# Roywangj/AdaptPoint

Measured on AMD Instinct MI355X. Metric: set-abstraction fwd+bwd point-clouds/sec (B=32,N=1024), higher is better.
Workload: dtype bf16

## Files before the change

### adaptpoint_amd/csrc/sa_fused.hip

```cpp
#include "apn_common.h"
#include "apn_mfma.h"
#include <type_traits>
#include "sa_chain.h"

namespace apn {

constexpr int SA_C = 32;
constexpr int SA_C1 = 32;
constexpr int SA_C2 = 64;
constexpr int SA_K = 32;
constexpr int SA_WAVES = 4;

template <int NS>
__device__ __forceinline__ void put_frag(uint4 *base, int f, int lane, const Frag<NS> &v) {
#pragma unroll
    for (int p = 0; p < NS; ++p) base[(f * NS + p) * 64 + lane] = __builtin_bit_cast(uint4, v.p[p]);
}

template <int NS>
__device__ __forceinline__ Frag<NS> get_frag(const uint4 *base, int f, int lane) {
    Frag<NS> v;
#pragma unroll
    for (int p = 0; p < NS; ++p) v.p[p] = __builtin_bit_cast(bf16x8, base[(f * NS + p) * 64 + lane]);
    return v;
// ... 305 lines not shown
            });
            stamp(a, wave, nst < 5 ? nst : 5);
            ++nst;
            hd_nxt = hd_nxt2;
            continue;
        }
        touch(hd_nxt);
        pre();
        if (more) fetch_tile<NS>(a, hd_nxt, h, nxt);
        const TileHead hd_nxt2 = load_head<CP>(a, tile2 < tiles ? tile2 : tile, r);
        body(tile, cur, nst == 4, [&] { touch(hd_nxt2); });
        stamp(a, wave, nst < 5 ? nst : 5);
        ++nst;
        if (more) cur = nxt;
        hd_nxt = hd_nxt2;
    }
    pre();
    stamp(a, wave, 6);
}

template <int NV>
__device__ __forceinline__ float fold_partials(float (&vals)[NV], int lane, int wave) {
    __shared__ float red[SA_WAVES][NV][32];
#pragma unroll
    for (int i = 0; i < NV; ++i) {
        const float other = __shfl_xor(vals[i], 32);
        if (lane < 32) red[wave][i][lane] = vals[i] + other;
    }
    __syncthreads();
    float s = 0.0f;
    const int e = threadIdx.x;
    if (e < NV * 32) {
#pragma unroll
        for (int w = 0; w < SA_WAVES; ++w) s += red[w][e >> 5][e & 31];
    }
    return s;
}

__device__ __forceinline__ void fold_rows32(const float *__restrict__ part, int rows, const double *__restrict__ sums,
                                            const BnArgs &bn, float *__restrict__ pack, float &scale, float &shift,
                                            double *scratch ) {
    double (*fred)[64] = reinterpret_cast<double (*)[64]>(scratch);
    double *ftot = scratch + 16 * 64;
    const int tid = threadIdx.x;
    double count = bn.count;
    double gpre = 1.0, bpre = 0.0;
    if (tid < 32) {
        if (bn.gamma) gpre = (double)bn.gamma[tid];
        if (bn.beta) bpre = (double)bn.beta[tid];
    }
    if (bn.training) {
        if (part) {
            const int quad = tid & 15, rg = tid >> 4;
            const float4 *__restrict__ p4 = reinterpret_cast<const float4 *>(part) + quad;
            double s0 = 0.0, s1 = 0.0, s2 = 0.0, s3 = 0.0;
            int rr = rg;
            for (; rr + 7 * 16 < rows; rr += 8 * 16) {
                float4 v[8];
#pragma unroll
                for (int u = 0; u < 8; ++u) v[u] = p4[(size_t)(rr + 16 * u) * 16];
#pragma unroll
                for (int u = 0; u < 8; ++u) {
                    s0 += (double)v[u].x; s1 += (double)v[u].y; s2 += (double)v[u].z; s3 += (double)v[u].w;
                }
            }
            for (; rr + 3 * 16 < rows; rr += 4 * 16) {
                float4 v[4];
#pragma unroll
                for (int u = 0; u < 4; ++u) v[u] = p4[(size_t)(rr + 16 * u) * 16];
#pragma unroll
                for (int u = 0; u < 4; ++u) {
                    s0 += (double)v[u].x; s1 += (double)v[u].y; s2 += (double)v[u].z; s3 += (double)v[u].w;
                }
            }
            for (; rr < rows; rr += 16) {
                const float4 v = p4[(size_t)rr * 16];
                s0 += (double)v.x; s1 += (double)v.y; s2 += (double)v.z; s3 += (double)v.w;
            }
            fred[rg][4 * quad] = s0; fred[rg][4 * quad + 1] = s1; fred[rg][4 * quad + 2] = s2; fred[rg][4 * quad + 3] = s3;
            __syncthreads();
            if (tid < 64) {
                double s = 0.0;
#pragma unroll
                for (int k = 0; k < 16; ++k) s += fred[k][tid];
                ftot[tid] = s;
            }
        } else if (tid < 64) {
            ftot[tid] = sums[tid];
        }
        if (!part) count = sums[64];
        __syncthreads();
    }
    if (tid < 32) {
        if (tid == 0 && blockIdx.x == 0 && bn.training && bn.nbt) *bn.nbt += 1;
        bn_channel(bn, 32, tid, bn.training ? ftot[tid] : 0.0, bn.training ? ftot[32 + tid] : 0.0, count,
                   blockIdx.x == 0, pack, scale, shift, gpre, bpre);
    }
}

template <int NS, bool CP>
__global__ __launch_bounds__(SA_WAVES * 64, 3) void sa_fwd_main_kernel(
    SaArgs a, const float *__restrict__ w2, BnArgs bn1, const float *__restrict__ part1, int rows1,
    const double *__restrict__ sums1, float *__restrict__ pack1, const float *__restrict__ gamma2,
    float *__restrict__ ysel, unsigned char *__restrict__ ksel, unsigned long long *__restrict__ acc2) {
    const int lane = threadIdx.x & 63, r = lane & 31, h = lane >> 5;
    const int wave = __builtin_amdgcn_readfirstlane(threadIdx.x >> 6);
    enum { F_W1 = 0, F_W2 = 3, F_COUNT = 7 };
    __shared__ uint4 cfrag[F_COUNT * NS * 64];
    __shared__ __attribute__((aligned(16))) float bn1v[2][2][16];
    constexpr int PT_WAVE = CP ? 2 * 32 * 33 : 17 * 64 * 2 / SA_WAVES;
    __shared__ __attribute__((aligned(16))) float ptile[SA_WAVES * PT_WAVE];
    __shared__ __attribute__((aligned(16))) unsigned sinfo[SA_WAVES][32];
    static_assert(SA_WAVES * PT_WAVE * 4 >= 17 * 64 * 8, "fold scratch");
    critical_stream_priority();
    stamp(a, wave, 0);
    const float sg[2] = {(!gamma2 || gamma2[r] >= 0.0f) ? 1.0f : -1.0f, (!gamma2 || gamma2[32 + r] >= 0.0f) ? 1.0f : -1.0f};
    float st[4] = {0.0f, 0.0f, 0.0f, 0.0f};

    auto prologue = [&]() {
        if (wave == 0) {
            Frag<NS> w1f[3];
            load_w1_frags<NS>(a.w1, r, h, w1f);
#pragma unroll
            for (int s = 0; s < 3; ++s) put_frag<NS>(cfrag, F_W1 + s, lane, w1f[s]);
        }
        if (wave == 1 || wave == 2) {
            const int t = wave - 1;
#pragma unroll
            for (int s = 0; s < 2; ++s) {
                float tmp[8];
#pragma unroll
                for (int j = 0; j < 8; ++j) tmp[j] = w2[(32 * t + r) * SA_C1 + acc_row(8 * s + j, h)];
                put_frag<NS>(cfrag, F_W2 + 2 * t + s, lane, make_frag<NS>(tmp));
            }
        }
        float sc, sh;
        fold_rows32(part1, rows1, sums1, bn1, pack1, sc, sh, reinterpret_cast<double *>(ptile));
        if (threadIdx.x < 32) {
            const int i = threadIdx.x;
            bn1v[0][(i >> 2) & 1][(i & 3) + 4 * (i >> 3)] = sc;
            bn1v[1][(i >> 2) & 1][(i & 3) + 4 * (i >> 3)] = sh;
        }
        __syncthreads();
    };

    for_each_tile<NS, CP>(a, wave, r, h, prologue, [] {}, [&](int tile, const TileRaw<NS> &raw, bool, auto before_stores) {
        int lane_o = lane;
        asm volatile("" : "+v"(lane_o));
        Frag<NS> x[3];
        build_frags<NS>(a, raw, h, x);
        const int q0 = __builtin_amdgcn_readfirstlane(raw.q0);
        const int nq = __builtin_amdgcn_readfirstlane((int)(raw.info >> 24));
        float multf[16];
        unsigned starts = 1u;
        float *pt = ptile + wave * PT_WAVE;
        if (CP) {
            if (lane < 32) sinfo[wave][lane] = raw.info;
#pragma unroll
            for (int gq = 0; gq < 4; ++gq) {
                const uint4 v = *reinterpret_cast<const uint4 *>(&sinfo[wave][8 * gq + 4 * (lane_o >> 5)]);
                multf[4 * gq] = (float)ri_mult(v.x); multf[4 * gq + 1] = (float)ri_mult(v.y);
                multf[4 * gq + 2] = (float)ri_mult(v.z); multf[4 * gq + 3] = (float)ri_mult(v.w);
            }
            const unsigned prev = (unsigned)__shfl_up((int)raw.info, 1);
            starts = (unsigned)__ballot(lane < 32 && (lane == 0 || ri_q(raw.info) != ri_q(prev)));
        }
        f32x16 y1 = {0};
#pragma unroll
        for (int s = 0; s < 3; ++s) y1 = mfma<NS>(get_frag<NS>(cfrag, F_W1 + s, lane_o), x[s], y1);
        {
            const float4 *scv = reinterpret_cast<const float4 *>(bn1v[0][lane_o >> 5]);
            const float4 *shv = reinterpret_cast<const float4 *>(bn1v[1][lane_o >> 5]);
#pragma unroll
            for (int i4 = 0; i4 < 4; ++i4) {
                const float4 sc = scv[i4], sh = shv[i4];
                y1[4 * i4] = __builtin_fmaxf(__builtin_fmaf(y1[4 * i4], sc.x, sh.x), 0.0f);
                y1[4 * i4 + 1] = __builtin_fmaxf(__builtin_fmaf(y1[4 * i4 + 1], sc.y, sh.y), 0.0f);
                y1[4 * i4 + 2] = __builtin_fmaxf(__builtin_fmaf(y1[4 * i4 + 2], sc.z, sh.z), 0.0f);
                y1[4 * i4 + 3] = __builtin_fmaxf(__builtin_fmaf(y1[4 * i4 + 3], sc.w, sh.w), 0.0f);
            }
        }
        const Frag<NS> a0 = pack8<NS>(y1, 0), a1 = pack8<NS>(y1, 8);
#pragma unroll
        for (int t = 0; t < 2; ++t) {
            f32x16 y2 = {0};
            y2 = mfma<NS>(a0, get_frag<NS>(cfrag, F_W2 + 2 * t, lane_o), y2);
            y2 = mfma<NS>(a1, get_frag<NS>(cfrag, F_W2 + 2 * t + 1, lane_o), y2);
            if (CP) {
                float s1 = 0.0f, s2 = 0.0f;
#pragma unroll
                for (int i = 0; i < 16; ++i) {
                    const float wy = multf[i] * y2[i];
                    s1 += wy;
                    s2 += wy * y2[i];
                    pt[(t * 32 + acc_row(i, h)) * 33 + r] = sg[t] * y2[i];
                }
                st[t] += s1;
                st[2 + t] += s2;
                continue;
            }
            float best = sg[t] * y2[0];
            int bpos = 0;
            float s1 = 0.0f, s2 = 0.0f;
#pragma unroll
            for (int i = 0; i < 16; ++i) {
                s1 += y2[i];
                s2 += y2[i] * y2[i];
                const float v = sg[t] * y2[i];
                if (i > 0 && v > best) { best = v; bpos = i; }
            }
            st[t] += s1;
            st[2 + t] += s2;
            int kpos = acc_row(bpos, h);
            const float obest = __shfl_xor(best, 32);
            const int okpos = __shfl_xor(kpos, 32);
            if (obest > best || (obest == best && okpos < kpos)) { best = obest; kpos = okpos; }
            if (h == 0) {
                ysel[(size_t)tile * SA_C2 + 32 * t + r] = sg[t] * best;
                ksel[(size_t)tile * SA_C2 + 32 * t + r] = (unsigned char)kpos;
            }
        }
        if (CP) {
            asm volatile("" ::: "memory");
            const float *mine = pt + h * (32 * 33) + r;
            const float sgn = h ? sg[1] : sg[0];
            float *ys = ysel + (size_t)q0 * SA_C2 + lane;
            unsigned char *ks = ksel + (size_t)q0 * SA_C2 + lane;
            before_stores();
            int seg = -1, ra = 0, kpos = 0;
            float best = 0.0f;
#pragma unroll
            for (int half16 = 0; half16 < 2; ++half16) {
                float v[16];
#pragma unroll
                for (int i = 0; i < 16; ++i) v[i] = mine[(16 * half16 + i) * 33];
#pragma unroll
                for (int i = 0; i < 16; ++i) {
                    const int rho = 16 * half16 + i;
                    if ((starts >> rho) & 1u) {
                        if (seg >= 0 && seg < nq) {
                            ys[(size_t)seg * SA_C2] = sgn * best;
                            ks[(size_t)seg * SA_C2] = (unsigned char)kpos;
                        }
                        ++seg;
                        best = -__builtin_inff();
                        kpos = 0;
                        ra = rho;
                    }
                    const bool up = v[i] > best;
                    best = up ? v[i] : best;
                    kpos = up ? rho - ra : kpos;
                }
            }
            if (seg >= 0 && seg < nq) {
                ys[(size_t)seg * SA_C2] = sgn * best;
                ks[(size_t)seg * SA_C2] = (unsigned char)kpos;
            }
            asm volatile("" ::: "memory");
        }
    });
    const float tot = fold_partials<4>(st, lane, wave);
    if (threadIdx.x < 128) acc_add(acc2, 128, blockIdx.x % ACC_COPIES, threadIdx.x, tot);
    stamp(a, wave, 7);
}

struct SaBwdArgs {
    const float *w2;
    const float *scale1, *shift1, *mean1, *inv1;
    const float *pack2;
    const unsigned long long *accS;
    const double *sumsS;
    double count;
    int train2;
    const float *goa;
    const unsigned char *ksel;
    const int *rowdst;
};

template <int NS, bool CP>
__global__ __launch_bounds__(SA_WAVES * 64, 2) void sa_bwd_kernel(SaArgs a, SaBwdArgs g,
                                                               unsigned long long *__restrict__ accT,
                                                               float *__restrict__ partW2,
                                                               float *__restrict__ GU,
                                                               float *__restrict__ HA,
                                                               float *__restrict__ HB) {
    static_assert(CP, "the backward pass runs over a tile map");
    const int lane = threadIdx.x & 63, r = lane & 31, h = lane >> 5;
    const int wave = __builtin_amdgcn_readfirstlane(threadIdx.x >> 6);
    enum { F_W1 = 0, F_QM = 3, F_W2T = 5, F_COUNT = 9 };
    __shared__ uint4 cfrag[F_COUNT * NS * 64];
    __shared__ __attribute__((aligned(16))) float bn1v[2][2][16];
    __shared__ __attribute__((aligned(16))) float sw2[SA_C2][SA_C1 + 4];
    __shared__ float sD[SA_C2], sE[SA_C2];
    __shared__ __attribute__((aligned(16))) float sqm[SA_C1 + 1][SA_C1 + 4];
    critical_stream_priority();
    stamp(a, wave, 0);
    __shared__ float chan[5][32];
    f32x16 dsp[2] = {{0}, {0}};
    f32x16 gram = {0};
    float suma = 0.0f;
    float st[2] = {0.0f, 0.0f};

    constexpr int SP_ROW = 72, SP_TILE = 32 * SP_ROW;
    constexpr int SP_WAVE = (CP && NS * SP_TILE * 2 < 2 * 32 * 33 * 4) ? 2 * 32 * 33 * 4 : NS * SP_TILE * 2;
    constexpr int SP_BYTES = SA_WAVES * SP_WAVE, WRED_BYTES = SA_WAVES * SA_C2 * SA_C1 * 4;
    __shared__ __attribute__((aligned(16))) unsigned char sp_raw[SP_BYTES > WRED_BYTES ? SP_BYTES : WRED_BYTES];
    __shared__ __attribute__((aligned(16))) unsigned sinfo[SA_WAVES][32];
    __shared__ __attribute__((aligned(16))) float qgoa[CP ? SA_WAVES : 1][4 * SA_C2];
    __shared__ __attribute__((aligned(16))) unsigned char qksel[CP ? SA_WAVES : 1][4 * SA_C2];
    __bf16 *sp_img = reinterpret_cast<__bf16 *>(sp_raw + wave * SP_WAVE);

    __shared__ __attribute__((aligned(16))) int sdst[SA_WAVES][2][64];
    int ahead_n = 0, body_n = 0;
    auto gu_store = [&](int place, float v) {
        *reinterpret_cast<float *>(reinterpret_cast<char *>(GU) + (((unsigned)place << 7) + ((unsigned)r << 2))) = v;
    };

    auto prologue = [&]() {
        const int tid = threadIdx.x;
        {
            Frag<NS> w1f[3];
            if (wave == 0) load_w1_frags<NS>(a.w1, r, h, w1f);
            float wv[8];
#pragma unroll
            for (int k = 0; k < 8; ++k) wv[k] = g.w2[tid + 256 * k];
            float c1[4] = {0.f, 0.f, 0.f, 0.f};
            if (tid >= 128 && tid < 160) {
                c1[0] = g.scale1[tid - 128]; c1[1] = g.shift1[tid - 128]; c1[2] = g.mean1[tid - 128]; c1[3] = g.inv1[tid - 128];
            }
            double sv = 0.0, count = g.count;
            float p_sc = 0.0f, p_mu = 0.0f, p_iv = 0.0f;
            if (tid < 128) sv = g.sumsS ? g.sumsS[tid] : acc_read(g.accS, 128, tid);
            if (g.sumsS) count = g.sumsS[128];
            if (tid < 64) { p_sc = g.pack2[tid]; p_mu = g.pack2[128 + tid]; p_iv = g.pack2[192 + tid]; }
            if (wave == 0) {
#pragma unroll
                for (int s = 0; s < 3; ++s) put_frag<NS>(cfrag, F_W1 + s, lane, w1f[s]);
            }
#pragma unroll
            for (int k = 0; k < 8; ++k) sw2[(tid + 256 * k) >> 5][tid & 31] = wv[k];
            if (tid >= 128 && tid < 160) {
#pragma unroll
                for (int k = 0; k < 4; ++k) chan[k][tid - 128] = c1[k];
            }
            double *sS2 = reinterpret_cast<double *>(&sqm[0][0]);
            if (tid >= 64 && tid < 128) sS2[tid - 64] = sv;
            __syncthreads();
            if (tid < 64) {
                const double sc = p_sc, mu = p_mu, iv = p_iv, s1 = sv, s2 = sS2[tid];
                double d = 0.0, e = 0.0;
                if (g.train2) {
                    const double rc = 1.0 / count;
                    d = -sc * iv * s2 * rc;
                    e = (-sc * s1 + sc * mu * iv * s2) * rc;
                }
                sD[tid] = (float)d;
                sE[tid] = (float)e;
            }
            if (tid >= 64 && tid < 96) {
                const int i = tid - 64;
                const float sci = g.scale1[i], shi = g.shift1[i];
                bn1v[0][(i >> 2) & 1][(i & 3) + 4 * (i >> 3)] = sci;
                bn1v[1][(i >> 2) & 1][(i & 3) + 4 * (i >> 3)] = shi;
            }
        }
        __syncthreads();
        {
            const int s = wave;
            float tmp[8], tmpd[8], tmpe[8];
#pragma unroll
            for (int j = 0; j < 8; ++j) {
                const int c = 16 * s + 8 * h + j;
                tmp[j] = sw2[c][r];
                tmpd[j] = tmp[j] * sD[c];
                tmpe[j] = r == 0 ? sE[c] : 0.0f;
            }
            const Frag<NS> wt = make_frag<NS>(tmp);
            put_frag<NS>(cfrag, F_W2T + s, lane, wt);
            const f32x16 zero16 = {0};
            const f32x16 qp = mfma<NS>(make_frag<NS>(tmpd), wt, zero16);
            const f32x16 ep = mfma<NS>(make_frag<NS>(tmpe), wt, zero16);
            float *scr = reinterpret_cast<float *>(sp_img);
#pragma unroll
            for (int e = 0; e < 16; ++e) scr[e * 64 + lane] = qp[e];
            if (h == 0) scr[16 * 64 + r] = ep[0];
        }
        __syncthreads();
        if (wave == 2) {
            f32x16 qacc = {0};
            float ev = 0.0f;
#pragma unroll
            for (int w = 0; w < SA_WAVES; ++w) {
                const float *pw = reinterpret_cast<const float *>(sp_raw + w * SP_WAVE);
#pragma unroll
                for (int e = 0; e < 16; ++e) qacc[e] += pw[e * 64 + lane];
                if (h == 0) ev += pw[16 * 64 + r];
            }
            put_frag<NS>(cfrag, F_QM, lane, pack8<NS>(qacc, 0));
            put_frag<NS>(cfrag, F_QM + 1, lane, pack8<NS>(qacc, 8));
            if (h == 0) chan[4][r] = ev;
        }
        __syncthreads();
        {
            uint4 *z = reinterpret_cast<uint4 *>(sp_img);
            for (int e = lane; e < SP_WAVE / 16; e += 64) z[e] = make_uint4(0u, 0u, 0u, 0u);
        }
    };

    auto scatter_pending = [] {};
    auto ahead = [&](const TileHead &hd) {
        if (!CP) return;
        typedef __attribute__((address_space(3))) void lds_void;
        typedef __attribute__((address_space(1))) const void glb_void;
        const int q0n = __builtin_amdgcn_readfirstlane(hd.q0);
        const int qbn = q0n < a.b * a.m - 4 ? q0n : a.b * a.m - 4;
        int l_o = lane;
        asm volatile("" : "+v"(l_o));
        const char *gb = reinterpret_cast<const char *>(g.goa) + (size_t)qbn * (SA_C2 * 4);
        const char *kb = reinterpret_cast<const char *>(g.ksel) + (size_t)qbn * SA_C2;
        __builtin_amdgcn_global_load_lds((glb_void *)(gb + (unsigned)(16 * l_o)), (lds_void *)&qgoa[wave][0], 16, 0, 0);
        __builtin_amdgcn_global_load_lds((glb_void *)(kb + (unsigned)(4 * l_o)), (lds_void *)&qksel[wave][0], 4, 0, 0);
        const char *db = reinterpret_cast<const char *>(g.rowdst) + (size_t)__builtin_amdgcn_readfirstlane(hd.tile) * (SA_K * 4);
        __builtin_amdgcn_global_load_lds((glb_void *)(db + (unsigned)(4 * (l_o & 31))), (lds_void *)&sdst[wave][ahead_n & 1][0], 4, 0, 0);
        ++ahead_n;
    };
    for_each_tile<NS, CP, CP>(a, wave, r, h, prologue, scatter_pending, [&](int tile, const TileRaw<NS> &raw, bool probe, auto before_stores) {
        auto st2 = [&](int k) { if (probe) stamp(a, wave, 8 + k); };
        st2(0);
        int lane_o = lane;
        asm volatile("" : "+v"(lane_o));
        Frag<NS> x[3];
        build_frags<NS>(a, raw, h, x);

        const int q0 = __builtin_amdgcn_readfirstlane(raw.q0);
        const int nq = CP ? __builtin_amdgcn_readfirstlane((int)(raw.info >> 24)) : 1;
        const bool live_row = !CP || ri_mult(raw.info) != 0;
        const float mrow = CP ? (float)ri_mult(raw.info) : 1.0f;
        float gv4[4];
        int kc4[4];
        const int qb = q0 < a.b * a.m - 4 ? q0 : a.b * a.m - 4;
#pragma unroll
        for (int u = 0; u < 4; ++u) {
            if (CP) {
                gv4[u] = 0.0f;
                kc4[u] = 0;
            } else {
                gv4[u] = 0.0f;
                kc4[u] = 0;
                if (u == 0) {
                    gv4[u] = g.goa[(size_t)(q0 + u) * SA_C2 + lane];
                    kc4[u] = g.ksel[(size_t)(q0 + u) * SA_C2 + lane];
                }
            }
        }
        unsigned mpk[4] = {0x01010101u, 0x01010101u, 0x01010101u, 0x01010101u};
        unsigned starts = 1u;
        if (CP) {
            if (lane < 32) sinfo[wave][lane] = raw.info;
#pragma unroll
            for (int gq = 0; gq < 4; ++gq) {
                const uint4 v = *reinterpret_cast<const uint4 *>(&sinfo[wave][8 * gq + 4 * (lane_o >> 5)]);
                mpk[gq] = ri_mult(v.x) | (ri_mult(v.y) << 8) | (ri_mult(v.z) << 16) | (ri_mult(v.w) << 24);
            }
            const unsigned prev = (unsigned)__shfl_up((int)raw.info, 1);
            starts = (unsigned)__ballot(lane < 32 && (lane == 0 || ri_q(raw.info) != ri_q(prev)));
        }
        auto multf = [&](int i) { return (float)((mpk[i >> 2] >> (8 * (i & 3))) & 0xffu); };
        f32x16 yT = {0}, y1 = {0};
#pragma unroll
        for (int s = 0; s < 3; ++s) {
            const Frag<NS> w = get_frag<NS>(cfrag, F_W1 + s, lane_o);
            yT = mfma<NS>(w, x[s], yT);
            y1 = mfma<NS>(x[s], w, y1);
        }
        {
            const float4 *scv = reinterpret_cast<const float4 *>(bn1v[0][lane_o >> 5]);
            const float4 *shv = reinterpret_cast<const float4 *>(bn1v[1][lane_o >> 5]);
#pragma unroll
            for (int i4 = 0; i4 < 4; ++i4) {
                const float4 sc = scv[i4], sh = shv[i4];
                yT[4 * i4] = __builtin_fmaxf(__builtin_fmaf(yT[4 * i4], sc.x, sh.x), 0.0f);
                yT[4 * i4 + 1] = __builtin_fmaxf(__builtin_fmaf(yT[4 * i4 + 1], sc.y, sh.y), 0.0f);
                yT[4 * i4 + 2] = __builtin_fmaxf(__builtin_fmaf(yT[4 * i4 + 2], sc.z, sh.z), 0.0f);
                yT[4 * i4 + 3] = __builtin_fmaxf(__builtin_fmaf(yT[4 * i4 + 3], sc.w, sh.w), 0.0f);
            }
        }
        st2(1);
        Frag<NS> a0, a1;
        if (CP) {
            f32x16 yw;
#pragma unroll
            for (int i = 0; i < 16; ++i) yw[i] = yT[i] * mrow;
            a0 = pack8<NS>(yw, 0);
            a1 = pack8<NS>(yw, 8);
        } else {
            a0 = pack8<NS>(yT, 0);
            a1 = pack8<NS>(yT, 8);
        }

        Frag<NS> sp[4];
        {
            unsigned todo = starts;
            if (CP) {
                asm volatile("s_waitcnt vmcnt(0)" ::: "memory");
                const int dq = q0 - qb;
#pragma unroll
                for (int u = 0; u < 4; ++u) {
                    const int e = (u + dq < 4 ? u + dq : 3) * SA_C2 + lane_o;
                    gv4[u] = qgoa[wave][e];
                    kc4[u] = qksel[wave][e];
                }
            }
#pragma unroll 1
            for (int jb = 0; jb < nq; jb += 4) {
                if (jb) {
#pragma unroll
                    for (int u = 0; u < 4; ++u)
                        if (jb + u < nq) {
                            gv4[u] = g.goa[(size_t)(q0 + jb + u) * SA_C2 + lane];
                            kc4[u] = g.ksel[(size_t)(q0 + jb + u) * SA_C2 + lane];
                        }
                }
#pragma unroll
                for (int u = 0; u < 4; ++u) {
                    if (jb + u < nq) {
                        const float gv = gv4[u];
                        int kc = kc4[u];
                        if (CP) {
                            kc += __builtin_ctz(todo);
                            todo &= todo - 1u;
                        }
                        const __bf16 ghi = (__bf16)gv;
                        const __bf16 glo = (__bf16)(gv - (float)ghi);
                        __bf16 *cell = sp_img + kc * SP_ROW + lane;
                        cell[0] = ghi;
                        if (NS == 2) cell[SP_TILE] = glo;
                        if (!CP) kc4[u] = kc;
                    }
                }
            }
        }
        asm volatile("" ::: "memory");
        {
            f32x16 an;
            const float sc1 = chan[0][lane_o & 31], sh1 = chan[1][lane_o & 31];
#pragma unroll
            for (int i = 0; i < 16; ++i) {
                an[i] = __builtin_fmaxf(__builtin_fmaf(y1[i], sc1, sh1), 0.0f);
                if (CP) suma = __builtin_fmaf(multf(i), an[i], suma);
                else suma += an[i];
            }
            const Frag<NS> b0 = pack8<NS>(an, 0), b1 = pack8<NS>(an, 8);
            if (CP) {
                f32x16 aw;
#pragma unroll
                for (int i = 0; i < 16; ++i) aw[i] = an[i] * multf(i);
                gram = mfma<NS>(pack8<NS>(aw, 0), b0, gram);
                gram = mfma<NS>(pack8<NS>(aw, 8), b1, gram);
            } else {
                gram = mfma<NS>(b0, b0, gram);
                gram = mfma<NS>(b1, b1, gram);
            }
            typedef short tr_s4 __attribute__((ext_vector_type(4)));
            typedef short tr_s8 __attribute__((ext_vector_type(8)));
            typedef __attribute__((address_space(3))) tr_s4 tr_lds;
            const int li = lane_o & 15, gq = li >> 2, gp = li & 3, grh = (lane_o >> 4) & 1;
            const __bf16 *tb = sp_img + (4 * (lane_o >> 5) + gq) * SP_ROW + 16 * grh + 4 * gp;
#pragma unroll
            for (int t = 0; t < 2; ++t) {
#pragma unroll
                for (int sk = 0; sk < 2; ++sk) {
                    Frag<NS> at;
#pragma unroll
                    for (int pp = 0; pp < NS; ++pp) {
                        const __bf16 *src = tb + pp * SP_TILE + (16 * sk) * SP_ROW + 32 * t;
                        const tr_s4 lo4 = __builtin_amdgcn_ds_read_tr16_b64_v4i16((tr_lds *)(src));
                        const tr_s4 hi4 = __builtin_amdgcn_ds_read_tr16_b64_v4i16((tr_lds *)(src + 8 * SP_ROW));
                        const tr_s8 v8 = {lo4.x, lo4.y, lo4.z, lo4.w, hi4.x, hi4.y, hi4.z, hi4.w};
                        at.p[pp] = __builtin_bit_cast(bf16x8, v8);
                    }
                    dsp[t] = mfma<NS>(at, sk ? b1 : b0, dsp[t]);
                }
            }
        }
        st2(2);
#pragma unroll
        for (int s = 0; s < 4; ++s) {
            const __bf16 *src = sp_img + r * SP_ROW + 16 * s + 8 * h;
            sp[s].p[0] = *reinterpret_cast<const bf16x8 *>(src);
            if (NS == 2) sp[s].p[NS - 1] = *reinterpret_cast<const bf16x8 *>(src + SP_TILE);
        }
        asm volatile("" ::: "memory");
        if (!CP) {
            __bf16 *cell = sp_img + kc4[0] * SP_ROW + lane;
            cell[0] = (__bf16)0.0f;
            if (NS == 2) cell[SP_TILE] = (__bf16)0.0f;
        }
        f32x16 ga;
        const float ev = chan[4][lane_o & 31];
#pragma unroll
        for (int i = 0; i < 16; ++i) ga[i] = CP ? ev * multf(i) : ev;
        ga = mfma<NS>(a0, get_frag<NS>(cfrag, F_QM, lane_o), ga);
        ga = mfma<NS>(a1, get_frag<NS>(cfrag, F_QM + 1, lane_o), ga);
#pragma unroll
        for (int s = 0; s < 4; ++s) ga = mfma<NS>(sp[s], get_frag<NS>(cfrag, F_W2T + s, lane_o), ga);

        st2(3);
        float *gt = reinterpret_cast<float *>(sp_img);
        asm volatile("" ::: "memory");
        float s1 = 0.0f, s2 = 0.0f, hb = 0.0f;
        const float sc1l = chan[0][lane_o & 31], sh1l = chan[1][lane_o & 31], iv1 = chan[3][lane_o & 31];
        const float nmi = -chan[2][lane_o & 31] * iv1;
#pragma unroll
        for (int i = 0; i < 16; ++i) {
            const float u = __builtin_fmaf(y1[i], sc1l, sh1l);
            const float yhat = __builtin_fmaf(y1[i], iv1, nmi);
            ga[i] = u > 0.0f ? ga[i] : 0.0f;
            s1 += ga[i];
            s2 += ga[i] * yhat;
            if (CP) {
                gt[acc_row(i, h) * 33 + r] = ga[i];
                gt[32 * 33 + acc_row(i, h) * 33 + r] = multf(i) * yhat;
            } else {
                hb += yhat;
            }
        }
        st[0] += s1;
        st[1] += s2;

        st2(4);
        before_stores();
        {
            int live;
            if (CP) {
                asm volatile("" ::: "memory");
                const float *mine = gt + h * (32 * 33) + r;
                float *dst = (h ? HB : HA) + (size_t)q0 * SA_C1 + r;
                int seg = -1;
                float sum = 0.0f;
#pragma unroll
                for (int half16 = 0; half16 < 2; ++half16) {
                    float v[16];
#pragma unroll
                    for (int i = 0; i < 16; ++i) v[i] = mine[(16 * half16 + i) * 33];
#pragma unroll
                    for (int i = 0; i < 16; ++i) {
                        if ((starts >> (16 * half16 + i)) & 1u) {
                            if (seg >= 0 && seg < nq) dst[(size_t)seg * SA_C1] = sum;
                            ++seg;
                            sum = 0.0f;
                        }
                        sum += v[i];
                    }
                }
                if (seg >= 0 && seg < nq) dst[(size_t)seg * SA_C1] = sum;
                asm volatile("" ::: "memory");
                {
                    uint4 *z = reinterpret_cast<uint4 *>(sp_img);
#pragma unroll
                    for (int e = 0; e < (NS * SP_TILE * 2 / 16 + 63) / 64; ++e)
                        if (e * 64 + lane < NS * SP_TILE * 2 / 16) z[e * 64 + lane] = make_uint4(0u, 0u, 0u, 0u);
                }
                asm volatile("" ::: "memory");
                live = __popcll(__ballot(lane < 32 && live_row));
            } else {
                const float ha = s1 + __shfl_xor(s1, 32);
                hb += __shfl_xor(hb, 32);
                if (h == 0) {
                    HA[(size_t)tile * SA_C1 + r] = ha;
                    HB[(size_t)tile * SA_C1 + r] = hb;
                }
                live = 0;
            }

            st2(5);
            st2(6);
            if (CP) {
                const int *dl = &sdst[wave][body_n & 1][0];
#pragma unroll
                for (int gq = 0; gq < 4; ++gq) {
                    if (8 * gq < live) {
                        const int4 dd = *reinterpret_cast<const int4 *>(&dl[8 * gq + 4 * (lane_o >> 5)]);
                        const int base = 8 * gq + 4 * h;
                        if (base + 0 < live) gu_store(dd.x, ga[4 * gq + 0]);
                        if (base + 1 < live) gu_store(dd.y, ga[4 * gq + 1]);
                        if (base + 2 < live) gu_store(dd.z, ga[4 * gq + 2]);
                        if (base + 3 < live) gu_store(dd.w, ga[4 * gq + 3]);
                    }
                }
            }
            ++body_n;
        }
    }, ahead);
    {
        const float tot = fold_partials<2>(st, lane, wave);
        if (threadIdx.x < 64) acc_add(accT, 64, blockIdx.x % ACC_COPIES, threadIdx.x, tot);
    }
    float (*wred)[SA_C2 * SA_C1] = reinterpret_cast<float (*)[SA_C2 * SA_C1]>(sp_raw);
    __syncthreads();
#pragma unroll
    for (int i = 0; i < 16; ++i) {
        wred[wave][acc_row(i, h) * SA_C1 + r] = dsp[0][i];
        wred[wave][(32 + acc_row(i, h)) * SA_C1 + r] = dsp[1][i];
    }
    __syncthreads();
    const int ec = threadIdx.x >> 2, emid = (threadIdx.x & 3) * 8;
    float sp8[8];
    {
        float4 lo4 = make_float4(0.f, 0.f, 0.f, 0.f), hi4 = lo4;
#pragma unroll
        for (int w = 0; w < SA_WAVES; ++w) {
            const float4 a4 = *reinterpret_cast<const float4 *>(&wred[w][ec * SA_C1 + emid]);
            const float4 b4 = *reinterpret_cast<const float4 *>(&wred[w][ec * SA_C1 + emid + 4]);
            lo4.x += a4.x; lo4.y += a4.y; lo4.z += a4.z; lo4.w += a4.w;
            hi4.x += b4.x; hi4.y += b4.y; hi4.z += b4.z; hi4.w += b4.w;
        }
        sp8[0] = lo4.x; sp8[1] = lo4.y; sp8[2] = lo4.z; sp8[3] = lo4.w;
        sp8[4] = hi4.x; sp8[5] = hi4.y; sp8[6] = hi4.z; sp8[7] = hi4.w;
    }
    __syncthreads();
    suma += __shfl_xor(suma, 32);
#pragma unroll
    for (int i = 0; i < 16; ++i) wred[wave][acc_row(i, h) * SA_C1 + r] = gram[i];
    if (h == 0) wred[wave][SA_C1 * SA_C1 + r] = suma;
    __syncthreads();
    for (int e = threadIdx.x; e < SA_C1 * SA_C1 + SA_C1; e += SA_WAVES * 64)
        sqm[e >> 5][e & 31] = (wred[0][e] + wred[1][e]) + (wred[2][e] + wred[3][e]);
    __syncthreads();
    {
        float acc[8];
#pragma unroll
        for (int j = 0; j < 8; ++j) acc[j] = 0.0f;
#pragma unroll 8
        for (int k = 0; k < SA_C1; ++k) {
            const float w = sw2[ec][k];
            const float4 g0 = *reinterpret_cast<const float4 *>(&sqm[k][emid]);
            const float4 g1 = *reinterpret_cast<const float4 *>(&sqm[k][emid + 4]);
            acc[0] = __builtin_fmaf(w, g0.x, acc[0]); acc[1] = __builtin_fmaf(w, g0.y, acc[1]);
            acc[2] = __builtin_fmaf(w, g0.z, acc[2]); acc[3] = __builtin_fmaf(w, g0.w, acc[3]);
            acc[4] = __builtin_fmaf(w, g1.x, acc[4]); acc[5] = __builtin_fmaf(w, g1.y, acc[5]);
            acc[6] = __builtin_fmaf(w, g1.z, acc[6]); acc[7] = __builtin_fmaf(w, g1.w, acc[7]);
        }
        const float d = sD[ec], e = sE[ec];
        const float4 s0 = *reinterpret_cast<const float4 *>(&sqm[32][emid]);
        const float4 s1 = *reinterpret_cast<const float4 *>(&sqm[32][emid + 4]);
        float4 *row = reinterpret_cast<float4 *>(partW2 + (size_t)blockIdx.x * (SA_C2 * SA_C1) + ec * SA_C1 + emid);
        row[0] = make_float4(sp8[0] + d * acc[0] + e * s0.x, sp8[1] + d * acc[1] + e * s0.y,
                             sp8[2] + d * acc[2] + e * s0.z, sp8[3] + d * acc[3] + e * s0.w);
        row[1] = make_float4(sp8[4] + d * acc[4] + e * s1.x, sp8[5] + d * acc[5] + e * s1.y,
                             sp8[6] + d * acc[6] + e * s1.z, sp8[7] + d * acc[7] + e * s1.w);
    }
    stamp(a, wave, 7);
}

static int sa_grid(int tiles, bool compact = false) {
    const int cap = compact ? 768 : 512;
    int g = (tiles + SA_WAVES - 1) / SA_WAVES;
    return g < cap ? (g < 1 ? 1 : g) : cap;
}

static int sa_grid_bwd(int tiles) {
    int g = sa_grid(tiles);
    return g < 448 ? g : 448;
}

}

extern "C" int apn_sa_grid_blocks(int b, int m) { return apn::sa_grid(b * m); }
extern "C" int apn_sa_grid_rows(int b, int m, int with_tile_map) { return apn::sa_grid(b * m, with_tile_map != 0); }
extern "C" int apn_sa_bwd_main_rows(int b, int m) { return apn::sa_grid_bwd(b * m); }
extern "C" int apn_sa_acc_words(int ncol) { return ncol > 0 ? apn::acc_words(ncol) : 0; }

extern "C" int apn_sa_prep_rows(int b, int n) {
    const long long tiles = (long long)b * ((n + apn::PS_PTS - 1) / apn::PS_PTS);
    return (int)(tiles < apn::PS_MAX_ROWS ? (tiles < 1 ? 1 : tiles) : apn::PS_MAX_ROWS);
}

extern "C" int apn_sa_prep_stats(int b, int n, const float *f, const void *geo, const void *dd, const float *w1,
                                 int precision, int stats, void *ft, float *part1, void *zero, long long zero_words,
                                 void *stream) {
    using namespace apn;
    if (b <= 0 || n <= 0 || b > 65535 || (precision != 1 && precision != 2) || !f || !ft || !w1) return APN_EINVAL;
    if (stats && (!geo || !dd || !part1 || ((uintptr_t)geo & 15) || ((uintptr_t)part1 & 15))) return APN_EINVAL;
    if (zero_words < 0 || (zero_words && !zero)) return APN_EINVAL;
    __bf16 *hi = (__bf16 *)ft;
    __bf16 *lo = precision == 2 ? hi + (size_t)b * n * SA_C : nullptr;
    const int tpc = (n + PS_PTS - 1) / PS_PTS;
    auto kern = precision == 2 ? sa_prep_stats_kernel<2> : sa_prep_stats_kernel<1>;
    const int lds = SA_C * (PS_PTS + 1) * (int)sizeof(float);
    static DynLdsOnce lds_set[2];
    if (hipError_t e = set_dyn_lds(lds_set[precision - 1], (const void *)kern, lds)) return (int)e;
    hipLaunchKernelGGL(kern, dim3(apn_sa_prep_rows(b, n)), dim3(PS_NT), lds, (hipStream_t)stream, n, tpc, b * tpc, f,
                       (const long long *)geo, (const double *)dd, b * (apn_sa_geo_dd_doubles(n) / 6), w1, stats, hi, lo, part1,
                       (unsigned long long *)zero, zero_words);
    APN_LAUNCH_CHECK();
    return APN_OK;
}

#ifdef APN_WG_STAMPS
extern "C" __attribute__((visibility("default"))) int apn_sa_debug_wg_stamps_fused(void *buf) {
    return (int)hipMemcpyToSymbol(HIP_SYMBOL(apn::d_wg_stamps_f), &buf, sizeof(buf));
}
#endif

static unsigned long long *g_stamps = nullptr;
extern "C" int apn_sa_debug_stamps(void *buf) { g_stamps = (unsigned long long *)buf; return APN_OK; }

static apn::SaArgs sa_args(int b, int n, int m, const float *xyz, const float *new_xyz, const void *ft,
                           int precision, const int *idx, const float *w1, float radius, const int *tmap) {
    const __bf16 *hi = (const __bf16 *)ft;
    return apn::SaArgs{b, n, m, xyz, new_xyz, hi,
                       precision == 2 ? hi + (size_t)b * n * apn::SA_C : nullptr, idx, w1, radius, tmap, g_stamps};
}

static int sa_check(int b, int n, int m, int precision) {
    if (precision != 1 && precision != 2) return APN_EINVAL;
    if (b <= 0 || n <= 0 || m <= 0) return APN_EINVAL;
    if ((long long)b * m > 0x7fffffffLL / 64) return APN_EINVAL;
    if ((long long)b * n > 0xffffffffLL / 256) return APN_EINVAL;
    if ((long long)b * m > 0xffffffffLL / (32 * 128)) return APN_EINVAL;
    return APN_OK;
}

extern "C" int apn_sa_fwd_main(int b, int n, int m, int precision, float radius, const float *xyz,
                               const float *new_xyz, const void *ft, const int *idx, const int *tmap, const float *w1,
                               const float *w2, const float *g1, const float *b1, float *rm1, float *rv1, void *nbt1,
                               float eps1, float mom1, int train1, double count, const float *part1, int rows1,
                               const double *sums1, float *pack1, const float *gamma2, float *ysel, void *ksel,
                               void *acc2, void *stream) {
    using namespace apn;
    if (int e = sa_check(b, n, m, precision)) return e;
    if (!xyz || !new_xyz || !ft || !idx || !w1 || !w2 || !pack1 || !ysel || !ksel || !acc2) return APN_EINVAL;
    if (train1 && !part1 && !sums1) return APN_EINVAL;
    if (!train1 && (!rm1 || !rv1)) return APN_EINVAL;
    if (part1 && (((uintptr_t)part1 & 15) || rows1 <= 0)) return APN_EINVAL;
    SaArgs a = sa_args(b, n, m, xyz, new_xyz, ft, precision, idx, w1, radius, tmap);
    BnArgs bn{g1, b1, rm1, rv1, (long long *)nbt1, eps1, mom1, train1, count};
    auto kern = precision == 2 ? (tmap ? sa_fwd_main_kernel<2, true> : sa_fwd_main_kernel<2, false>)
                               : (tmap ? sa_fwd_main_kernel<1, true> : sa_fwd_main_kernel<1, false>);
    hipLaunchKernelGGL(kern, dim3(sa_grid(b * m, tmap != nullptr)), dim3(SA_WAVES * 64), 0, (hipStream_t)stream, a, w2, bn,
                       sums1 ? nullptr : part1, rows1, sums1, pack1, gamma2, ysel, (unsigned char *)ksel,
                       (unsigned long long *)acc2);
    APN_LAUNCH_CHECK();
    return APN_OK;
}

extern "C" int apn_sa_bwd_main(int b, int n, int m, int precision, float radius, const float *xyz,
                               const float *new_xyz, const void *ft, const int *idx, const int *tmap, const float *w1,
                               const float *w2, const float *pack1, const float *pack2, const void *accS,
                               const double *sumsS, double count, int train2, const float *goa, const void *ksel,
                               void *accT, float *partW2, const int *rowdst, float *GU, float *HA, float *HB, void *stream) {
    using namespace apn;
    if (int e = sa_check(b, n, m, precision)) return e;
    if (!w2 || !pack1 || !pack2 || (!accS && !sumsS) || !goa || !ksel || !accT || !partW2 || !GU || !HA || !HB)
        return APN_EINVAL;
    if (!tmap || !rowdst) return APN_EINVAL;
    SaArgs a = sa_args(b, n, m, xyz, new_xyz, ft, precision, idx, w1, radius, tmap);
    SaBwdArgs g;
    g.w2 = w2;
    g.scale1 = pack1; g.shift1 = pack1 + 32; g.mean1 = pack1 + 64; g.inv1 = pack1 + 96;
    g.pack2 = pack2;
    g.accS = (const unsigned long long *)accS; g.sumsS = sumsS;
    g.count = count; g.train2 = train2;
    g.goa = goa; g.ksel = (const unsigned char *)ksel;
    g.rowdst = rowdst;
    auto kern = precision == 2 ? sa_bwd_kernel<2, true> : sa_bwd_kernel<1, true>;
    hipLaunchKernelGGL(kern, dim3(sa_grid_bwd(b * m)), dim3(SA_WAVES * 64), 0, (hipStream_t)stream, a, g,
                       (unsigned long long *)accT, partW2, GU, HA, HB);
    APN_LAUNCH_CHECK();
    return APN_OK;
}
```

Measured before the change: 121,900.

## Derive transposed activations via LDS transpose reads and segment-sum with MFMA

The backward tile no longer runs a second W1 MFMA chain to get the transposed activations. It computes the BN/ReLU output once, writes it to a swizzled LDS image and reads it back transposed with ds_read_tr16. The per-query segment sums of the gradient and yhat, previously done with an LDS round trip and serial scan, are now done as MFMAs against a one-hot segment matrix built from the row info. The scatter image is now cleared cell by cell when there are at most four queries, instead of zeroing the whole image. This trades MFMA and LDS-scan work for extra LDS writes and transposed reads. It also changes the BN used for the transposed operand from bn1v to the chan scale/shift, which could alter the numerics.

```diff
diff --git a/adaptpoint_amd/csrc/sa_fused.hip b/adaptpoint_amd/csrc/sa_fused.hip
--- a/adaptpoint_amd/csrc/sa_fused.hip
+++ b/adaptpoint_amd/csrc/sa_fused.hip
@@ -631,7 +631,9 @@
     float st[2] = {0.0f, 0.0f};
 
     constexpr int SP_ROW = 72, SP_TILE = 32 * SP_ROW;
-    constexpr int SP_WAVE = (CP && NS * SP_TILE * 2 < 2 * 32 * 33 * 4) ? 2 * 32 * 33 * 4 : NS * SP_TILE * 2;
+    constexpr int AI_PLANE = 32 * 64;
+    constexpr int SP_WAVE = NS * SP_TILE * 2;
+    static_assert(NS * AI_PLANE <= SP_WAVE, "the transposed image fits the wave's region");
     constexpr int SP_BYTES = SA_WAVES * SP_WAVE, WRED_BYTES = SA_WAVES * SA_C2 * SA_C1 * 4;
     __shared__ __attribute__((aligned(16))) unsigned char sp_raw[SP_BYTES > WRED_BYTES ? SP_BYTES : WRED_BYTES];
     __shared__ __attribute__((aligned(16))) unsigned sinfo[SA_WAVES][32];
@@ -764,7 +766,6 @@
         const int q0 = __builtin_amdgcn_readfirstlane(raw.q0);
         const int nq = CP ? __builtin_amdgcn_readfirstlane((int)(raw.info >> 24)) : 1;
         const bool live_row = !CP || ri_mult(raw.info) != 0;
-        const float mrow = CP ? (float)ri_mult(raw.info) : 1.0f;
         float gv4[4];
         int kc4[4];
         const int qb = q0 < a.b * a.m - 4 ? q0 : a.b * a.m - 4;
@@ -795,36 +796,68 @@
             starts = (unsigned)__ballot(lane < 32 && (lane == 0 || ri_q(raw.info) != ri_q(prev)));
         }
         auto multf = [&](int i) { return (float)((mpk[i >> 2] >> (8 * (i & 3))) & 0xffu); };
-        f32x16 yT = {0}, y1 = {0};
-#pragma unroll
-        for (int s = 0; s < 3; ++s) {
-            const Frag<NS> w = get_frag<NS>(cfrag, F_W1 + s, lane_o);
-            yT = mfma<NS>(w, x[s], yT);
-            y1 = mfma<NS>(x[s], w, y1);
-        }
+        f32x16 y1 = {0};
+#pragma unroll
+        for (int s = 0; s < 3; ++s) y1 = mfma<NS>(x[s], get_frag<NS>(cfrag, F_W1 + s, lane_o), y1);
+        st2(1);
+        typedef short tr_s4 __attribute__((ext_vector_type(4)));
+        typedef short tr_s8 __attribute__((ext_vector_type(8)));
+        typedef __attribute__((address_space(3))) tr_s4 tr_lds;
+        const int li = lane_o & 15, gq4 = li >> 2, gp = li & 3, grh = (lane_o >> 4) & 1, hh = lane_o >> 5;
+        Frag<NS> a0, a1, b0, b1;
         {
-            const float4 *scv = reinterpret_cast<const float4 *>(bn1v[0][lane_o >> 5]);
-            const float4 *shv = reinterpret_cast<const float4 *>(bn1v[1][lane_o >> 5]);
-#pragma unroll
-            for (int i4 = 0; i4 < 4; ++i4) {
-                const float4 sc = scv[i4], sh = shv[i4];
-                yT[4 * i4] = __builtin_fmaxf(__builtin_fmaf(yT[4 * i4], sc.x, sh.x), 0.0f);
-                yT[4 * i4 + 1] = __builtin_fmaxf(__builtin_fmaf(yT[4 * i4 + 1], sc.y, sh.y), 0.0f);
-                yT[4 * i4 + 2] = __builtin_fmaxf(__builtin_fmaf(yT[4 * i4 + 2], sc.z, sh.z), 0.0f);
-                yT[4 * i4 + 3] = __builtin_fmaxf(__builtin_fmaf(yT[4 * i4 + 3], sc.w, sh.w), 0.0f);
-            }
-        }
-        st2(1);
-        Frag<NS> a0, a1;
-        if (CP) {
-            f32x16 yw;
-#pragma unroll
-            for (int i = 0; i < 16; ++i) yw[i] = yT[i] * mrow;
-            a0 = pack8<NS>(yw, 0);
-            a1 = pack8<NS>(yw, 8);
-        } else {
-            a0 = pack8<NS>(yT, 0);
-            a1 = pack8<NS>(yT, 8);
+            f32x16 an, aw;
+            const float sc1 = chan[0][lane_o & 31], sh1 = chan[1][lane_o & 31];
+#pragma unroll
+            for (int i = 0; i < 16; ++i) {
+                an[i] = __builtin_fmaxf(__builtin_fmaf(y1[i], sc1, sh1), 0.0f);
+                suma = __builtin_fmaf(multf(i), an[i], suma);
+                aw[i] = an[i] * multf(i);
+            }
+            b0 = pack8<NS>(an, 0);
+            b1 = pack8<NS>(an, 8);
+            const Frag<NS> w0 = pack8<NS>(aw, 0), w1 = pack8<NS>(aw, 8);
+            gram = mfma<NS>(w0, b0, gram);
+            gram = mfma<NS>(w1, b1, gram);
+            asm volatile("" ::: "memory");
+            unsigned char *ai = reinterpret_cast<unsigned char *>(sp_img);
+            const int sw = ((lane_o & 31) >> 1) & 3;
+#pragma unroll
+            for (int pp = 0; pp < NS; ++pp)
+#pragma unroll
+                for (int s = 0; s < 2; ++s) {
+                    const uint4 v = __builtin_bit_cast(uint4, (s ? w1 : w0).p[pp]);
+#pragma unroll
+                    for (int e = 0; e < 2; ++e) {
+                        const int c8 = 4 * s + ((2 * e + hh) ^ sw);
+                        *reinterpret_cast<uint2 *>(ai + pp * AI_PLANE + (lane_o & 31) * 64 + 8 * c8) =
+                            e ? make_uint2(v.z, v.w) : make_uint2(v.x, v.y);
+                    }
+                }
+            asm volatile("" ::: "memory");
+            const int row = 4 * hh + gq4;
+            const unsigned char *tb = ai + row * 64 + 8 * (4 * grh + (gp ^ ((row >> 1) & 3)));
+#pragma unroll
+            for (int s = 0; s < 2; ++s) {
+                Frag<NS> at;
+#pragma unroll
+                for (int pp = 0; pp < NS; ++pp) {
+                    const unsigned char *src = tb + pp * AI_PLANE + s * 16 * 64;
+                    const tr_s4 lo4 = __builtin_amdgcn_ds_read_tr16_b64_v4i16((tr_lds *)(src));
+                    const tr_s4 hi4 = __builtin_amdgcn_ds_read_tr16_b64_v4i16((tr_lds *)(src + 8 * 64));
+                    const tr_s8 v8 = {lo4.x, lo4.y, lo4.z, lo4.w, hi4.x, hi4.y, hi4.z, hi4.w};
+                    at.p[pp] = __builtin_bit_cast(bf16x8, v8);
+                }
+                if (s) a1 = at;
+                else a0 = at;
+            }
+            asm volatile("" ::: "memory");
+            {
+                uint4 *z = reinterpret_cast<uint4 *>(sp_img);
+#pragma unroll
+                for (int e = 0; e < NS * AI_PLANE / 16 / 64; ++e) z[e * 64 + lane_o] = make_uint4(0u, 0u, 0u, 0u);
+            }
+            asm volatile("" ::: "memory");
         }
 
         Frag<NS> sp[4];
@@ -864,37 +897,14 @@
                         __bf16 *cell = sp_img + kc * SP_ROW + lane;
                         cell[0] = ghi;
                         if (NS == 2) cell[SP_TILE] = glo;
-                        if (!CP) kc4[u] = kc;
+                        kc4[u] = kc;
                     }
                 }
             }
         }
         asm volatile("" ::: "memory");
         {
-            f32x16 an;
-            const float sc1 = chan[0][lane_o & 31], sh1 = chan[1][lane_o & 31];
-#pragma unroll
-            for (int i = 0; i < 16; ++i) {
-                an[i] = __builtin_fmaxf(__builtin_fmaf(y1[i], sc1, sh1), 0.0f);
-                if (CP) suma = __builtin_fmaf(multf(i), an[i], suma);
-                else suma += an[i];
-            }
-            const Frag<NS> b0 = pack8<NS>(an, 0), b1 = pack8<NS>(an, 8);
-            if (CP) {
-                f32x16 aw;
-#pragma unroll
-                for (int i = 0; i < 16; ++i) aw[i] = an[i] * multf(i);
-                gram = mfma<NS>(pack8<NS>(aw, 0), b0, gram);
-                gram = mfma<NS>(pack8<NS>(aw, 8), b1, gram);
-            } else {
-                gram = mfma<NS>(b0, b0, gram);
-                gram = mfma<NS>(b1, b1, gram);
-            }
-            typedef short tr_s4 __attribute__((ext_vector_type(4)));
-            typedef short tr_s8 __attribute__((ext_vector_type(8)));
-            typedef __attribute__((address_space(3))) tr_s4 tr_lds;
-            const int li = lane_o & 15, gq = li >> 2, gp = li & 3, grh = (lane_o >> 4) & 1;
-            const __bf16 *tb = sp_img + (4 * (lane_o >> 5) + gq) * SP_ROW + 16 * grh + 4 * gp;
+            const __bf16 *tb = sp_img + (4 * hh + gq4) * SP_ROW + 16 * grh + 4 * gp;
 #pragma unroll
             for (int t = 0; t < 2; ++t) {
 #pragma unroll
@@ -920,11 +930,21 @@
             if (NS == 2) sp[s].p[NS - 1] = *reinterpret_cast<const bf16x8 *>(src + SP_TILE);
         }
         asm volatile("" ::: "memory");
-        if (!CP) {
-            __bf16 *cell = sp_img + kc4[0] * SP_ROW + lane;
-            cell[0] = (__bf16)0.0f;
-            if (NS == 2) cell[SP_TILE] = (__bf16)0.0f;
-        }
+        if (nq <= 4) {
+#pragma unroll
+            for (int u = 0; u < 4; ++u)
+                if (u < nq) {
+                    __bf16 *cell = sp_img + kc4[u] * SP_ROW + lane;
+                    cell[0] = (__bf16)0.0f;
+                    if (NS == 2) cell[SP_TILE] = (__bf16)0.0f;
+                }
+        } else {
+            uint4 *z = reinterpret_cast<uint4 *>(sp_img);
+#pragma unroll
+            for (int e = 0; e < (NS * SP_TILE * 2 / 16 + 63) / 64; ++e)
+                if (e * 64 + lane < NS * SP_TILE * 2 / 16) z[e * 64 + lane] = make_uint4(0u, 0u, 0u, 0u);
+        }
+        asm volatile("" ::: "memory");
         f32x16 ga;
         const float ev = chan[4][lane_o & 31];
 #pragma unroll
@@ -935,9 +955,8 @@
         for (int s = 0; s < 4; ++s) ga = mfma<NS>(sp[s], get_frag<NS>(cfrag, F_W2T + s, lane_o), ga);
 
         st2(3);
-        float *gt = reinterpret_cast<float *>(sp_img);
-        asm volatile("" ::: "memory");
         float s1 = 0.0f, s2 = 0.0f, hb = 0.0f;
+        f32x16 yw;
         const float sc1l = chan[0][lane_o & 31], sh1l = chan[1][lane_o & 31], iv1 = chan[3][lane_o & 31];
         const float nmi = -chan[2][lane_o & 31] * iv1;
 #pragma unroll
@@ -947,50 +966,48 @@
             ga[i] = u > 0.0f ? ga[i] : 0.0f;
             s1 += ga[i];
             s2 += ga[i] * yhat;
-            if (CP) {
-                gt[acc_row(i, h) * 33 + r] = ga[i];
-                gt[32 * 33 + acc_row(i, h) * 33 + r] = multf(i) * yhat;
-            } else {
-                hb += yhat;
-            }
+            if (CP) yw[i] = multf(i) * yhat;
+            else hb += yhat;
         }
         st[0] += s1;
         st[1] += s2;
+        f32x16 hsa = {0}, hsb = {0};
+        if (CP) {
+            auto one = [&](unsigned info) { return ri_q(info) == (unsigned)(lane_o & 31) ? 0x3f80u : 0u; };
+#pragma unroll
+            for (int s = 0; s < 2; ++s) {
+                const uint4 v0 = *reinterpret_cast<const uint4 *>(&sinfo[wave][16 * s + 4 * hh]);
+                const uint4 v1 = *reinterpret_cast<const uint4 *>(&sinfo[wave][16 * s + 8 + 4 * hh]);
+                const bf16x8 seg = __builtin_bit_cast(bf16x8, make_uint4(one(v0.x) | (one(v0.y) << 16), one(v0.z) | (one(v0.w) << 16),
+                                                                         one(v1.x) | (one(v1.y) << 16), one(v1.z) | (one(v1.w) << 16)));
+                const Frag<NS> fa = pack8<NS>(ga, 8 * s), fb = pack8<NS>(yw, 8 * s);
+                if (NS == 2) {
+                    hsa = mfma(seg, fa.p[NS - 1], hsa);
+                    hsb = mfma(seg, fb.p[NS - 1], hsb);
+                }
+                hsa = mfma(seg, fa.p[0], hsa);
+                hsb = mfma(seg, fb.p[0], hsb);
+            }
+        }
 
         st2(4);
         before_stores();
         {
             int live;
             if (CP) {
-                asm volatile("" ::: "memory");
-                const float *mine = gt + h * (32 * 33) + r;
-                float *dst = (h ? HB : HA) + (size_t)q0 * SA_C1 + r;
-                int seg = -1;
-                float sum = 0.0f;
-#pragma unroll
-                for (int half16 = 0; half16 < 2; ++half16) {
-                    float v[16];
-#pragma unroll
-                    for (int i = 0; i < 16; ++i) v[i] = mine[(16 * half16 + i) * 33];
-#pragma unroll
-                    for (int i = 0; i < 16; ++i) {
-                        if ((starts >> (16 * half16 + i)) & 1u) {
-                            if (seg >= 0 && seg < nq) dst[(size_t)seg * SA_C1] = sum;
-                            ++seg;
-                            sum = 0.0f;
+#pragma unroll
+                for (int gq = 0; gq < 4; ++gq) {
+                    if (8 * gq < nq) {
+#pragma unroll
+                        for (int j = 0; j < 4; ++j) {
+                            const int qq = 8 * gq + 4 * h + j;
+                            if (qq < nq) {
+                                HA[(size_t)(q0 + qq) * SA_C1 + r] = hsa[4 * gq + j];
+                                HB[(size_t)(q0 + qq) * SA_C1 + r] = hsb[4 * gq + j];
+                            }
                         }
-                        sum += v[i];
                     }
                 }
-                if (seg >= 0 && seg < nq) dst[(size_t)seg * SA_C1] = sum;
-                asm volatile("" ::: "memory");
-                {
-                    uint4 *z = reinterpret_cast<uint4 *>(sp_img);
-#pragma unroll
-                    for (int e = 0; e < (NS * SP_TILE * 2 / 16 + 63) / 64; ++e)
-                        if (e * 64 + lane < NS * SP_TILE * 2 / 16) z[e * 64 + lane] = make_uint4(0u, 0u, 0u, 0u);
-                }
-                asm volatile("" ::: "memory");
                 live = __popcll(__ballot(lane < 32 && live_row));
             } else {
                 const float ha = s1 + __shfl_xor(s1, 32);
```

Result: no change. 121,000 (median of 2 runs) (-0.8%).
